# MattAgostini/ECE1782-Smith-Waterman-CUDA

Measured on AMD Instinct MI355X. Metric: GCUPS (DP cell updates/s) query-vs-SwissProt, 1/2/4/8 MI355X; bit-exact scores, higher is better.
Workload: dtype fp16

## Files before the change

ece1782-smith-waterman-cuda_amd/csrc/sw_capi.cpp:

```cpp
#include <algorithm>
#include <cmath>
#include <atomic>
#include <cstdio>
#include <cstdlib>
#include <cstring>
#include <memory>
#include <new>
#include <numeric>
#include <string>
#include <unordered_map>
#include <vector>

#include "sw_dbfile.h"
#include "sw_host.h"
#include "sw_pack.h"
#include "sw_parallel.h"
#include "sw_plan.h"
#include "sw_synth_host.h"

using swk::DevPtr;
using swk::Event;
using swk::HostPtr;
using swk::parallel_for;
using swk::Stream;
// ... 598 lines not shown
    const uint8_t* codes = nullptr;
    const sw_scoring* sc = nullptr;
    const sw_pssm* pssm = nullptr;
    int go = 0, ge = 0;
    int32_t qlen = 0;
};
QuerySrc seq_src(const uint8_t* q, int32_t qlen, const sw_scoring* sc) {
    QuerySrc s;
    s.codes = q;
    s.qlen = qlen;
    s.sc = sc;
    return s;
}
QuerySrc pssm_src(const sw_pssm* p, int32_t go, int32_t ge) {
    QuerySrc s;
    s.pssm = p;
    s.qlen = p ? p->qlen : 0;
    s.go = go;
    s.ge = ge;
    return s;
}
int check_pssm(const sw_handle* h, const sw_pssm* p, int go, int ge) {
    if (!h || !p) return fail(SW_E_INVALID, "null argument");
    if (p->h->device != h->device) return fail(SW_E_INVALID, "the PSSM was created on another handle's device");
    return check_gaps(go, ge);
}

struct Profiles {
    int8_t* dev = nullptr;
    int32_t stride = 0;
    size_t off8 = 0;
    size_t off16 = 0;
    size_t intra_off = 0;
    size_t total = 0;
    int slot = 0;
};

int build_profiles(sw_handle* h, const QuerySrc& src, const int8_t* mat, int go, bool affine,
                   int32_t qpad_inter, bool want16, int ri, int32_t qpad_intra, int32_t* const (&reset)[10],
                   Profiles* P) {
    const uint8_t* q = src.codes;
    const int32_t qlen = src.qlen;
    for (int32_t i = 0; i < qlen && !src.pssm; ++i)
        if (q[i] >= SW_ALPHABET) return fail(SW_E_INVALID, "query residue code out of range (use sw_encode)");
    const int bias = affine ? 0 : go;
    P->stride = static_cast<int32_t>(round_up(std::max<int32_t>(qpad_inter, 16), 16));
    const size_t n = static_cast<size_t>(swk::kProfileRows) * P->stride;
    size_t at = 0;
    auto take = [&](size_t bytes) {
        const size_t o = at;
        at = round_up(static_cast<int64_t>(at + bytes), 256);
        return o;
    };
    P->off8 = take(n);
    P->off16 = want16 ? take(2 * n) : 0;
    const int rip = swk::intra_rip(ri);
    const size_t intra_bytes = ri ? static_cast<size_t>(qpad_intra / (swk::kLanes * ri)) * swk::intra_chunk_bytes(ri) : 0;
    P->intra_off = take(intra_bytes);
    P->total = at;
    P->slot = h->prof_next;
    sw_handle::ProfSlot& S = h->prof[h->prof_next];
    h->prof_next = (h->prof_next + 1) % sw_handle::kProfSlots;
    if (S.pending) HIPCHECK(hipEventSynchronize(S.last_end));
    S.pending = false;
    if (P->total > S.dcap) {
        if (S.d.get()) {
            HIPCHECK(hipStreamSynchronize(h->stream.get()));
            if (S.tail_pending) HIPCHECK(hipEventSynchronize(S.tail_read.get()));
            S.tail_pending = false;
            S.d.reset();
        }
        S.dcap = std::max<size_t>(P->total, 1 << 16);
        HIPCHECK(swk::dev_alloc(S.d, S.dcap));
    }
    P->dev = S.d.get();
    if (S.tail_pending) {
        HIPCHECK(hipStreamWaitEvent(h->stream.get(), S.tail_read.get(), 0));
        S.tail_pending = false;
    }
    if (src.pssm) {
        swk::PssmProfileArgs a{};
        a.p8 = S.d.get() + P->off8;
        a.p16 = want16 ? reinterpret_cast<int16_t*>(S.d.get() + P->off16) : nullptr;
        a.pin = ri ? S.d.get() + P->intra_off : nullptr;
        a.stride = P->stride;
        a.qlen = qlen;
        a.bias = bias;
        a.ri = ri;
        a.rip = rip;
        a.qpad_intra = ri ? qpad_intra : 0;
        a.rows = std::max(P->stride, a.qpad_intra);
        for (int k = 0; k < 10; ++k) a.reset[k] = reset[k];
        a.pssm = src.pssm->d.get();
        a.ld = src.pssm->ld;
        HIPCHECK(swk::launch_build_profile_pssm(a, h->stream.get()));
        S.last_end = h->ev[3].get();
        S.pending = true;
        h->open_slot = P->slot;
        return SW_OK;
    }
    swk::ProfileArgs a{};
    a.p8 = S.d.get() + P->off8;
    a.p16 = want16 ? reinterpret_cast<int16_t*>(S.d.get() + P->off16) : nullptr;
    a.pin = ri ? S.d.get() + P->intra_off : nullptr;
    a.stride = P->stride;
    a.qlen = qlen;
    a.bias = bias;
    a.ri = ri;
    a.rip = rip;
    a.qpad_intra = ri ? qpad_intra : 0;
    for (int k = 0; k < 10; ++k) a.reset[k] = reset[k];
    std::memcpy(a.mat, mat, 625);
    const int32_t rows = std::max(P->stride, a.qpad_intra);
    for (int32_t r0 = 0; r0 < rows; r0 += swk::kProfQueryChunk) {
        a.row0 = r0;
        a.row1 = std::min(rows, r0 + swk::kProfQueryChunk);
        const int32_t nq = std::max(0, std::min(a.row1, qlen) - r0);
        if (nq) std::memcpy(a.q, q + r0, static_cast<size_t>(nq));
        HIPCHECK(swk::launch_build_profile(a, h->stream.get()));
        for (auto& p : a.reset) p = nullptr;
    }
    S.last_end = h->ev[3].get();
    S.pending = true;
    h->open_slot = P->slot;
    return SW_OK;
}

const sw_db::LptTable* lpt_table(sw_db* db, const swplan::ScanPlan& p) {
    const sw_opts& O = db->h->opts;
    const bool tri = p.ntri != 0;
    for (const auto& t : db->lay.lpt_tables)
        if (t.qpad == p.qpad_inter && t.rows == p.lpt_rows && t.qpad_intra == p.qpad_intra2 && t.ri == p.ri2 &&
            t.npair == p.npair && t.group == p.nquad && t.tail == p.ntail && t.pipe_opt == O.lpt_pipe &&
            t.affine == p.affine && t.tri == tri && t.tail_opt == O.lpt_pipe_tail)
            return &t;
    const swplan::LptPlan pl = swplan::lpt_plan(plan_view(db), p.qpad_inter, p.lpt_rows, p.qpad_intra2, p.ri2, p.npair,
                                                p.nquad, p.ntail, p.affine, tri);
    sw_db::LptTable t{p.qpad_inter, p.lpt_rows, p.qpad_intra2, p.ri2, p.npair, p.nquad, p.ntail,
                      static_cast<int32_t>(pl.order.size()), p.affine, tri, pl.npipe, O.lpt_pipe, pl.pipe_tail,
                      O.lpt_pipe_tail, DevPtr<int32_t>{}, pl.cost};
    const size_t bytes = pl.order.size() * sizeof(int32_t);
    hipError_t e = swk::dev_alloc(t.d_order, bytes);
    if (e == hipSuccess) e = hipMemcpy(t.d_order.get(), pl.order.data(), bytes, hipMemcpyHostToDevice);
// ... 177 lines not shown
    c.par = h->parity;
    h->parity ^= 1;
    if (h->tail_pending[c.par]) {
        HIPCHECK(hipStreamWaitEvent(h->stream.get(), h->tail_done[c.par].get(), 0));
        h->tail_pending[c.par] = false;
    }
    if (p.drain && (rc = join_tails(h))) return rc;
    if (db->lay.d_rescue.get()) {
        c.listA = db->lay.d_rescue.get() + c.par * rstride;
        c.listB = c.listA + db->shape.nblocks + 1;
        c.maxA = c.listA + 2 * (db->shape.nblocks + 1);
        c.headA = c.maxA + 2;
        if (p.lpt && h->opts.lpt_persist != 0) c.lpt_next = c.maxA + 1;
    }
    if (db->lay.d_lrescue.get()) {
        c.list1 = db->lay.d_lrescue.get() + c.par * lstride;
        c.list2 = c.list1 + db->shape.nlong + 1;
        c.head1 = c.list2 + db->shape.nlong + 1;
    }
    c.deferred = !p.drain && defer && (!(p.multi_inter || p.multi_intra) || ensure_rbnd(db, p.affine, p.intra_x2));
    return SW_OK;
}

int scan_profiles(Scan& c, const QuerySrc& src, const int8_t* mat) {
    const swplan::ScanPlan& p = c.plan;
    const bool d = p.drain;
    int32_t* const cA = (p.rescue && c.db->shape.nblocks) ? c.listA : nullptr;
    int32_t* const c1 = p.intra_x2 ? c.list1 : nullptr;
    int32_t* const reset[10] = {cA, (cA && p.f16) ? c.listB : nullptr, (cA && p.f16) ? c.maxA : nullptr, c1,
                                c1 ? c.list2 : nullptr, d ? c.headA : nullptr, d ? c.headA + 1 : nullptr,
                                d ? c.head1 : nullptr, d ? c.head1 + 1 : nullptr, c.lpt_next};
    const int rc = build_profiles(c.h, src, mat, c.sc.go, p.affine,
                                  std::max({p.qpad_inter, p.qpad_rescue, p.qpad_coop, p.qpad_list, p.qpad_intra2}),
                                  p.shape.x2s || p.intra_x2, p.ri, p.qpad_intra, reset, &c.P);
    c.h->evpool[c.h->nscans - 1].merged = p.lpt;
    return rc;
}

int inter_args(Scan& c) {
    sw_db* db = c.db;
    const swplan::ScanPlan& p = c.plan;
    const int go = c.sc.go, ge = c.sc.ge;
    swk::InterArgs& a = c.a;
    a.residues = db->lay.d_res.get();
    a.blk_off = db->lay.d_blk_off.get();
    a.blk_groups = db->lay.d_blk_groups.get();
    a.blk_cols = db->lay.d_blk_cols.get();
    a.lane_ids = db->lay.d_lane_ids.get();
    a.nblocks = static_cast<int32_t>(db->shape.nblocks);
    a.prof = c.P.dev + (p.shape.x2s ? c.P.off16 : c.P.off8);
    a.prof_stride = c.P.stride;
    a.qpad = p.qpad_inter;
    a.gap_open = go;
    a.gap_extend = ge;
    a.bnd_h = db->lay.d_bnd_h.get();
    a.bnd_f = db->lay.d_bnd_f.get();
    a.scores = c.scores;
    if (c.h->opts.trace_file[0]) {
        if (!db->lay.h_trace.get()) {
            db->lay.trace_entries = static_cast<size_t>(2 * db->shape.nblocks + db->shape.nlong + 8);
            HIPCHECK(swk::host_alloc(db->lay.h_trace, 32 * db->lay.trace_entries, hipHostMallocMapped));
            std::memset(db->lay.h_trace.get(), 0, 32 * db->lay.trace_entries);
        }
        HIPCHECK(hipHostGetDevicePointer(reinterpret_cast<void**>(&a.trace), db->lay.h_trace.get(), 0));
    }
    if (p.rescue) {
        a.rescue_count = c.listA;
        a.rescue_list = c.listA + 1;
        if (p.f16) a.rescue_max = c.maxA;
        const swplan::CellRange cr = swplan::cell_range(-128, c.sc.max_s, go, ge);
        a.sat_limit = cr.sat_limit;
        std::copy(std::begin(cr.step), std::end(cr.step), a.f16_step);
        a.f16_gog = cr.gog;
        a.f16_zero = cr.step[0];
        std::copy(std::begin(cr.diff), std::end(cr.diff), a.f16_diff);
    }
    a.re_last = p.re_last;
    if (p.lpt) {
        a.blk_first = p.npair;
        a.blk_quad = p.nquad;
        a.blk_tri = p.ntri ? 1 : 0;
        a.blk_tail = static_cast<int32_t>(db->shape.nblocks) - p.ntail;
    } else if (p.npair) {
        a.blk_base = p.nr;
        a.blk_first = std::max(p.npair, p.nr);
    } else {
        a.blk_first = p.ncoop;
    }
    return SW_OK;
}

void intra_args(Scan& c) {
    const sw_db* db = c.db;
    swk::IntraArgs& ia = c.ia;
    ia.residues = db->lay.d_lres.get();
    ia.subj_off = db->lay.d_loff.get();
    ia.subj_len = db->lay.d_llen.get();
    ia.subj_id = db->lay.d_lid.get();
    ia.nsubj = static_cast<int32_t>(db->shape.nlong);
    ia.prof = c.P.dev + c.P.intra_off;
    ia.qpad = c.plan.qpad_intra;
    ia.gap_open = c.sc.go;
    ia.gap_extend = c.sc.ge;
    ia.bnd_h = db->lay.d_lbnd_h.get();
    ia.bnd_f = db->lay.d_lbnd_f.get();
    ia.scores = c.scores;
}

void intra_x2_args(Scan& c) {
    const swplan::ScanPlan& p = c.plan;
// ... 1144 lines not shown
```

ece1782-smith-waterman-cuda_amd/csrc/sw_inter_x2.hip:

```cpp
#include <algorithm>

#include "sw_int32.h"
#include "sw_intra_x2.h"
#include "sw_kernels.h"

namespace swk {

typedef short s2 __attribute__((ext_vector_type(2)));
typedef unsigned short u2 __attribute__((ext_vector_type(2)));

__device__ __forceinline__ s2 as_s2(uint32_t x) { return __builtin_bit_cast(s2, x); }
__device__ __forceinline__ uint32_t as_u32(s2 x) { return __builtin_bit_cast(uint32_t, x); }
__device__ __forceinline__ s2 max2(s2 a, s2 b) { return __builtin_elementwise_max(a, b); }
__device__ __forceinline__ s2 usub2(s2 a, u2 g) {
    return __builtin_bit_cast(s2, __builtin_elementwise_sub_sat(__builtin_bit_cast(u2, a), g));
}

__host__ __device__ constexpr int x2_row_dwords(int R) { return (R / 4) % 2 == 1 ? R : R + 4; }

constexpr int kImgCodes = kPadCode + 1;

template <int R>
struct __attribute__((aligned(16))) X2Lds {
    static constexpr int kImg = kImgCodes * x2_row_dwords(R);
    uint32_t lo[kImg];
    uint32_t hi[kImg];
};
static_assert(sizeof(X2Lds<32>) % 16 == 0 && sizeof(X2Lds<48>) % 16 == 0, "image alignment");

template <int N>
__device__ __forceinline__ uint32_t word(const int4 (&v)[N], int w) {
    const int4 q = v[w >> 2];
    switch (w & 3) {
        case 0: return static_cast<uint32_t>(q.x);
        case 1: return static_cast<uint32_t>(q.y);
        case 2: return static_cast<uint32_t>(q.z);
        default: return static_cast<uint32_t>(q.w);
    }
}

template <int SG>
__device__ __forceinline__ void load_codes(uint32_t (&w)[SG / 4], const uint8_t* p, bool valid) {
    if (valid) {
        if constexpr (SG == 16) {
            const int4 v = *reinterpret_cast<const int4*>(p);
            w[0] = v.x; w[1] = v.y; w[2] = v.z; w[3] = v.w;
        } else if constexpr (SG == 8) {
            const int2 v = *reinterpret_cast<const int2*>(p);
            w[0] = v.x; w[1] = v.y;
        } else {
            w[0] = *reinterpret_cast<const uint32_t*>(p);
        }
    } else {
#pragma unroll
        for (int q = 0; q < SG / 4; ++q) w[q] = 0x19191919u;
    }
}

__device__ __forceinline__ uint32_t code_of(const uint32_t* w, int jj) { return (w[jj >> 2] >> (8 * (jj & 3))) & 0xffu; }

template <uint32_t RB>
// ... 26 lines not shown
__device__ __forceinline__ void load_bnd(uint32_t (&v)[SG], const uint32_t* bnd, uint64_t i) {
    if constexpr (AFFINE) {
        load_pairs<SG>(v, reinterpret_cast<const int32_t*>(bnd) + i);
    } else {
        const uint16_t* p = reinterpret_cast<const uint16_t*>(bnd) + i;
        uint32_t w[SG / 2];
        if constexpr (SG == 8) {
            const int4 t = *reinterpret_cast<const int4*>(p);
            w[0] = t.x; w[1] = t.y; w[2] = t.z; w[3] = t.w;
        } else {
            static_assert(SG == 4, "sub-group width");
            const int2 t = *reinterpret_cast<const int2*>(p);
            w[0] = t.x; w[1] = t.y;
        }
#pragma unroll
        for (int q = 0; q < SG; ++q) v[q] = w[q / 2];
    }
}
template <int SG, bool AFFINE>
__device__ __forceinline__ void store_bnd(uint32_t* bnd, uint64_t i, const uint32_t (&hb)[SG]) {
    if constexpr (AFFINE) {
        store_pairs<SG>(reinterpret_cast<int32_t*>(bnd) + i, hb);
    } else {
        uint16_t* p = reinterpret_cast<uint16_t*>(bnd) + i;
        uint32_t w[SG / 2];
#pragma unroll
        for (int q = 0; q < SG / 2; ++q) w[q] = lo_lo(hb[2 * q], hb[2 * q + 1]);
        if constexpr (SG == 8) *reinterpret_cast<int4*>(p) = make_int4(w[0], w[1], w[2], w[3]);
        else *reinterpret_cast<int2*>(p) = make_int2(w[0], w[1]);
    }
}


template <int R, bool F16>
__device__ __forceinline__ void stage_x2s(X2Lds<R>& L, const int16_t* __restrict__ prof, int stride, int s0,
                                          int lane, int bias, int bias0, int img, int hi0 = R) {
    constexpr int RD = x2_row_dwords(R);
    constexpr int PER = kImgCodes * (R / 8);
    constexpr uint32_t one = 1u;
    const int n = img < 0 ? 2 * PER : PER;
    for (int t = lane; t < n; t += kLanes) {
        const int im = img < 0 ? t / PER : img;
        const int u = img < 0 ? t % PER : t;
        const int c = u / (R / 8);
        const int k = u % (R / 8);
        const int16_t* src = prof + static_cast<size_t>(c) * stride + s0 + im * hi0 + 8 * k;
        int4 v;
        if (im && (hi0 & 7)) {
            const int2 v0 = *reinterpret_cast<const int2*>(src), v1 = *reinterpret_cast<const int2*>(src + 4);
            v = make_int4(v0.x, v0.y, v1.x, v1.y);
        } else {
            v = *reinterpret_cast<const int4*>(src);
        }
        const uint32_t w[4] = {static_cast<uint32_t>(v.x), static_cast<uint32_t>(v.y), static_cast<uint32_t>(v.z),
                               static_cast<uint32_t>(v.w)};
        uint32_t o[8];
#pragma unroll
        for (int e = 0; e < 4; ++e) {
            const int s0v = static_cast<int16_t>(w[e] & 0xffffu), s1v = static_cast<int16_t>(w[e] >> 16);
            const int b0 = (F16 && k % 2 == 0 && e == 0) ? bias0 : 0;
            const uint32_t a0 = static_cast<uint32_t>(s0v) & 0xffffu, a1 = static_cast<uint32_t>(s1v) & 0xffffu;
            if constexpr (F16) {
                const uint32_t w0 = static_cast<uint32_t>(s0v + bias + b0), w1 = static_cast<uint32_t>(s1v + bias);
                o[2 * e] = im ? w0 << 16 : w0;
                o[2 * e + 1] = im ? w1 << 16 : w1;
            } else {
                o[2 * e] = im ? (a0 << 16) | one : a0 | (one << 16);
                o[2 * e + 1] = im ? (a1 << 16) | one : a1 | (one << 16);
            }
        }
        int4* d = reinterpret_cast<int4*>((im ? L.hi : L.lo) + c * RD + 8 * k);
        d[0] = make_int4(o[0], o[1], o[2], o[3]);
        d[1] = make_int4(o[4], o[5], o[6], o[7]);
    }
}


typedef int v4i __attribute__((ext_vector_type(4)));
typedef __attribute__((address_space(3))) const v4i lds_int4;

__device__ __forceinline__ uint32_t lds_addr(const void* p) {
    return static_cast<uint32_t>(reinterpret_cast<uintptr_t>(p));
}

template <int N>
__device__ __forceinline__ void read_x2a(int4 (&pl)[N], int4 (&ph)[N], uint32_t& aa, uint32_t& ab, int k,
                                         uint32_t dep) {
    asm volatile("" : "+v"(aa), "+v"(ab) : "v"(dep));
    lds_int4* a = reinterpret_cast<lds_int4*>(static_cast<uintptr_t>(aa)) + N * k;
    lds_int4* b = reinterpret_cast<lds_int4*>(static_cast<uintptr_t>(ab)) + N * k;
#pragma unroll
    for (int q = 0; q < N; ++q) {
        pl[q] = __builtin_bit_cast(int4, a[q]);
        ph[q] = __builtin_bit_cast(int4, b[q]);
    }
}

typedef _Float16 h2 __attribute__((ext_vector_type(2)));

template <bool F16>
struct PkCell;

template <>
struct PkCell<false> {
    using V = s2;
    static __device__ __forceinline__ V from(uint32_t x) { return as_s2(x); }
// ... 154 lines not shown
};
__device__ __forceinline__ void pair_wait(const int* prog, int wave, int need) {
    while (__hip_atomic_load(prog + wave, __ATOMIC_ACQUIRE, __HIP_MEMORY_SCOPE_WORKGROUP) < need)
        __builtin_amdgcn_s_sleep(1);
}

template <int R, int SG, bool AFFINE, bool F16, bool PAIR, int CR = 16, bool CHAIN = false, int RL = R>
__device__ __forceinline__ void x2s_pass(const InterArgs& a, X2Lds<R>& L, uint32_t ncols, uint64_t base, int lane,
                                         int s0, Best<F16>& best, const int4* ring_in, int4* ring_out,
                                         int* tick, const PairSync* ps = nullptr, int chain_passes = 1) {
    static_assert(!(CHAIN && PAIR), "chained passes: single-wave blocks only");
    constexpr int CQ = CR / 4;
    constexpr int NCH = R / CR;
    constexpr int STEPS = SG * NCH;
    using P = PkCell<F16>;
    using V = typename P::V;
    const int16_t* prof16 = reinterpret_cast<const int16_t*>(a.prof);
    const u2 go2 = {static_cast<unsigned short>(a.gap_open), static_cast<unsigned short>(a.gap_open)};
    const u2 ge2 = {static_cast<unsigned short>(a.gap_extend), static_cast<unsigned short>(a.gap_extend)};
    uint32_t* bnd = reinterpret_cast<uint32_t*>(a.bnd_h);
    static_assert(!F16 || (R % kRowGroup == 0 && SG <= 8), "fp16 row groups");
    h2 gog_h = {}, reb_h = {}, grp_h = {};
    if constexpr (F16) {
        gog_h = __builtin_bit_cast(h2, a.f16_gog);
        static_assert(SG == 4 || SG == 8, "rebase constants");
        reb_h = __builtin_bit_cast(h2, a.f16_diff[SG == 4 ? 0 : 1]);
        grp_h = __builtin_bit_cast(h2, a.f16_diff[2]);
    }
    const bool first = (s0 == 0);
    const bool last = (s0 + 2 * R >= a.qpad);
    const uint32_t npass = CHAIN ? static_cast<uint32_t>(chain_passes) : 1u;
    const bool chain_last = CHAIN && static_cast<int>(npass) * 2 * R >= a.qpad;
    const uint32_t total = npass * ncols;
    const int sbias = F16 ? (AFFINE ? 2 : 1) * a.gap_extend : 0;
    const int gbias0 = F16 ? -kRowGroup * a.gap_extend : 0;
    const uint32_t dtop0 = F16 ? a.f16_step[SG - 2 + kRowGroup] : 0u;
    constexpr bool kSh = RL < R;
    if constexpr (kSh) asm volatile("" : "+v"(lane));
    static_assert(!kSh || (RL == R - 4 && !CHAIN), "rows per strip: R, or R - 4 outside a chain");
    static_assert((R - 4 - 1) % kRowGroup == 11, "the short strip's bottom row: 4 ge under the last row's bias");
    h2 dsh_h = {};
    if constexpr (F16) dsh_h = __builtin_bit_cast(h2, a.f16_diff[0]);
    stage_x2s<R, F16>(L, prof16, a.prof_stride, s0, lane, sbias, gbias0, -1, RL);
    __builtin_amdgcn_fence(__ATOMIC_RELEASE, "workgroup");
    __builtin_amdgcn_wave_barrier();
    __builtin_amdgcn_fence(__ATOMIC_ACQUIRE, "workgroup");

    V H[R];
    V E[AFFINE ? R : 1];
#pragma unroll
    for (int r = 0; r < R; ++r) H[r] = P::from(F16 && r < RL ? a.f16_step[r % kRowGroup + SG - 1] : 0u);
#pragma unroll
    for (int r = 0; r < (AFFINE ? R : 1); ++r) E[r] = P::from(F16 ? a.f16_zero : 0u);
    uint32_t dtop = dtop0;
    uint32_t dl_h[SG], dl_f[SG];
    uint32_t bin[SG], bin_n[SG];
    uint32_t bz[SG];
    uint32_t rc[SG / 4], rp[SG / 4], rn[SG / 4];
#pragma unroll
    for (int q = 0; q < SG; ++q) {
        bz[q] = !F16 ? 0u
                     : AFFINE ? lo_lo(a.f16_step[kRowGroup - 1 + q], a.f16_step[kRowGroup + q])
                              : lo_lo(a.f16_step[kRowGroup - 1 + q], a.f16_step[kRowGroup - 1 + q]);
        dl_h[q] = F16 ? a.f16_step[kRowGroup - 1 + q] : 0u;
        dl_f[q] = F16 ? a.f16_step[kRowGroup + q] : 0u;
        bin[q] = bz[q];
        bin_n[q] = 0;
    }
#pragma unroll
    for (int q = 0; q < SG / 4; ++q) rp[q] = 0x19191919u;
    load_codes<SG>(rc, a.residues + base, true);
    constexpr bool kPairFlags = pair_flags<AFFINE>();
    auto wait_in = [&](uint32_t x) {
        if constexpr (PAIR && kPairFlags)
            pair_wait(ps->prog, ps->pred, ps->pred_base + min(static_cast<int>(x) + 2, ps->S));
    };
    if (!first) {
        wait_in(0);
        if (PAIR && ring_in) ring_load<SG>(bin, ring_in, 0, lane);
        else load_bnd<SG, AFFINE>(bin, bnd, base);
    }
    int4 PL[2][CQ], PH[2][CQ];
    constexpr uint32_t RB = x2_row_dwords(R) * 4;
    const uint32_t blo = lds_addr(L.lo), bhi = lds_addr(L.hi);
    uint32_t aa = code_row<RB>(rc, 0, blo), ab = bhi + kPadCode * RB;
    read_x2a<CQ>(PL[0], PH[0], aa, ab, 0, 0);

    uint32_t lo_p = 0, lo_c = 0;
    bool t2 = false;
    for (uint32_t col0 = 0; col0 <= total; col0 += SG) {
        const bool has_next = col0 + SG <= total;
        const bool next_lo = col0 + SG < total;
        const uint32_t ncol = col0 + SG;
        const bool wrap = CHAIN && lo_c + SG == ncols;
        const uint32_t nreal = CHAIN ? (wrap ? 0u : lo_c + SG) : ncol;
        const bool next_first = CHAIN ? (lo_p == 0 && !wrap) : first;
        const uint64_t noff = (nreal >> 4) * kGroupBytes + (nreal & 15);
        const bool t1 = CHAIN && lo_c == 0 && lo_p > 0 && lo_p < npass;
        const bool next_t1 = CHAIN && wrap && next_lo;
        const bool next_t2 = t1;
        if (t1) {
            stage_x2s<R, F16>(L, prof16, a.prof_stride, static_cast<int>(lo_p) * 2 * R, lane, sbias, gbias0, 0);
#pragma unroll
            for (int r = 0; r < R; ++r) {
                H[r] = P::from(__builtin_amdgcn_perm(P::bits(H[r]), F16 ? a.f16_step[r % kRowGroup + SG - 1] : 0u,
                                                     0x07060100u));
                if constexpr (AFFINE) E[r] = P::from(__builtin_amdgcn_perm(P::bits(E[r]), F16 ? a.f16_zero : 0u, 0x07060100u));
            }
            dtop = __builtin_amdgcn_perm(dtop, dtop0, 0x07060100u);
        }
        if (t2) {
            stage_x2s<R, F16>(L, prof16, a.prof_stride, static_cast<int>(lo_p) * 2 * R, lane, sbias, gbias0, 1);
#pragma unroll
            for (int r = 0; r < R; ++r) {
                H[r] = P::from(__builtin_amdgcn_perm(F16 ? a.f16_step[r % kRowGroup + SG - 1] : 0u, P::bits(H[r]),
                                                     0x07060100u));
                if constexpr (AFFINE) E[r] = P::from(__builtin_amdgcn_perm(F16 ? a.f16_zero : 0u, P::bits(E[r]), 0x07060100u));
            }
            dtop = __builtin_amdgcn_perm(dtop0, dtop, 0x07060100u);
        }
        if (t1 || t2) {
            __builtin_amdgcn_fence(__ATOMIC_RELEASE, "workgroup");
            __builtin_amdgcn_wave_barrier();
            __builtin_amdgcn_fence(__ATOMIC_ACQUIRE, "workgroup");
            aa = code_row<RB>(rc, 0, blo);
            ab = code_row<RB>(rp, 0, bhi);
            read_x2a<CQ>(PL[0], PH[0], aa, ab, 0, 0);
        }
        if (next_t1) {
            __builtin_amdgcn_fence(__ATOMIC_RELEASE, "workgroup");
            __builtin_amdgcn_fence(__ATOMIC_ACQUIRE, "workgroup");
        }
        if (has_next) {
            load_codes<SG>(rn, a.residues + base + noff, next_lo);
            if (!next_first && next_lo) {
                wait_in(ncol / SG);
                if (PAIR && ring_in) ring_load<SG>(bin_n, ring_in, (ncol / SG) % kRingSlots, lane);
                else load_bnd<SG, AFFINE>(bin_n, bnd, base + noff);
            }
        }
        if constexpr (F16) {
#pragma unroll
            for (int r = 0; r < R; ++r) {
                if (r < RL) H[r] = isub(H[r], reb_h);
                if constexpr (AFFINE)
                    if (r < RL) E[r] = isub(E[r], reb_h);
            }
            dtop -= P::bits(reb_h);
        }
        auto cell = [&](const int r, const int jj, V& up, V& diag, V& f, const V slo, const V shi) {
            if constexpr (F16 && !AFFINE) {
                const int rg = r % kRowGroup;
                if (rg == 0 && r > 0) up = isub(up, grp_h);
                const h2 t = max3h(H[r], up, iadd(iadd(slo, shi), diag));
                const h2 h = __builtin_elementwise_maximum(t, __builtin_bit_cast(h2, a.f16_step[rg + jj]));
                h2& acc = best.acc[rg + jj];
                if (jj & 1) {
                    if (rg + 1 < kRowGroup) acc = max3h(acc, h, H[r + 1]);
                    else acc = __builtin_elementwise_maximum(acc, h);
                } else if (rg == 0) {
                    acc = __builtin_elementwise_maximum(acc, h);
                }
                diag = H[r];
                H[r] = h;
                up = h;
            } else if constexpr (!AFFINE) {
                const s2 h = usub2(max2(max2(H[r], up), slo * shi + diag), go2);
                diag = H[r];
                H[r] = h;
                up = h;
                best.v = max2(best.v, h);
            } else if constexpr (!F16) {
                const s2 h = max2(max2(E[r], f), slo * shi + diag);
                const s2 n = usub2(h, go2);
                E[r] = max2(usub2(E[r], ge2), n);
                f = max2(usub2(f, ge2), n);
                diag = H[r];
                H[r] = h;
                up = h;
                best.v = max2(best.v, h);
            }
        };
        auto cell_d = [&](const int r, const int jj, V& up, V& diag, V& f, const V d) {
          if constexpr (F16 && AFFINE) {
            const int rg = r % kRowGroup;
            if (rg == 0 && r > 0) f = isub(f, grp_h);
            const h2 h = max3h(E[r], f, d);
            const h2 m = isub(h, gog_h);
            E[r] = __builtin_elementwise_maximum(E[r], m);
            f = max3h(f, m, __builtin_bit_cast(h2, a.f16_step[rg + jj + 1]));
            h2& acc = best.acc[rg + jj];
            if (jj & 1) {
                if (rg + 1 < kRowGroup) acc = max3h(acc, h, H[r + 1]);
                else acc = __builtin_elementwise_maximum(acc, h);
            } else if (rg == 0) {
                acc = __builtin_elementwise_maximum(acc, h);
            }
            diag = H[r];
            H[r] = h;
            up = h;
          }
        };
        auto col_done = [&](const V up, const V f, const int jj) {
            if constexpr (kSh && F16) {
                dl_h[jj] = P::bits(iadd(up, dsh_h));
                if constexpr (AFFINE) dl_f[jj] = P::bits(iadd(f, dsh_h));
            } else {
                dl_h[jj] = P::bits(up);
                if constexpr (AFFINE) dl_f[jj] = P::bits(f);
            }
        };
        auto col_start = [&](V& up, V& diag, V& f, const int jj) {
            const uint32_t u = (AFFINE || jj % 2 == 0) ? lo_lo(bin[jj], dl_h[jj]) : hi_lo(bin[jj], dl_h[jj]);
            up = P::from(u);
            if constexpr (F16 && !AFFINE) up = isub(up, grp_h);
            diag = P::from(dtop);
            dtop = u;
            if constexpr (AFFINE) f = P::from(hi_lo(bin[jj], dl_f[jj]));
            if constexpr (F16) f = isub(f, grp_h);
        };
        V up = P::from(0u), diag = P::from(0u), f = P::from(0u);
#pragma unroll
        for (int t = 0; t < STEPS; ++t) {
            const int jj = t / NCH;
            const int k = t % NCH;
            const uint32_t dep = P::bits(k == 0 ? H[R - 1] : H[CR * k - 1]);
            if (t + 1 < STEPS) {
                const int jn = (t + 1) / NCH, kn = (t + 1) % NCH;
                if (kn == 0) {
                    aa = code_row<RB>(rc, jn, blo);
// ... 465 lines not shown
```

ece1782-smith-waterman-cuda_amd/csrc/sw_kernels.h:

```cpp
#pragma once

#include <hip/hip_runtime.h>
#include <stdint.h>

#include <string>

#include "sw_amd.h"

namespace swk {

int set_error(int code, const std::string& msg);

constexpr int kLanes = 64;
constexpr int kGroupCols = 16;
constexpr int kGroupBytes = kLanes * kGroupCols;
constexpr int kProfileRows = 32;
constexpr int kPadCode = 25;
constexpr uint8_t kStored[26] = {11, 1, 5, 2, 22, 6, 14, 12, 23, 9, 10, 0, 24, 7, 4, 15, 3, 21, 8, 13, 16, 17, 18, 19, 20, 25};
constexpr uint8_t kCodeOf[26] = {11, 1, 3, 16, 14, 2, 5, 13, 18, 9, 10, 0, 7, 19, 6, 15, 20, 21, 22, 23, 24, 17, 4, 8, 12, 25};
constexpr int kWavesPerWG = 4;
constexpr int kIntraSteps = 40;

template <int SG>
struct Residues {
    uint32_t w[SG / 4];
    __device__ __forceinline__ void load(const uint8_t* p) {
        if constexpr (SG == 16) {
            const int4 v = *reinterpret_cast<const int4*>(p);
            w[0] = v.x; w[1] = v.y; w[2] = v.z; w[3] = v.w;
        } else if constexpr (SG == 8) {
            const int2 v = *reinterpret_cast<const int2*>(p);
            w[0] = v.x; w[1] = v.y;
        } else {
            w[0] = *reinterpret_cast<const uint32_t*>(p);
        }
    }
    __device__ __forceinline__ uint32_t code(int jj) const { return (w[jj >> 2] >> (8 * (jj & 3))) & 0xffu; }
};

struct InterArgs {
    const uint8_t* residues;
    const uint64_t* blk_off;
    const uint32_t* blk_groups;
    const uint32_t* blk_cols;
    const int32_t* lane_ids;
    int32_t nblocks;
    const int8_t* prof;
    int32_t prof_stride;
    int32_t qpad;
    int32_t gap_open;
    int32_t gap_extend;
    int32_t* bnd_h;
    int32_t* bnd_f;
    int32_t* scores;
    int32_t* rescue_list;
    int32_t* rescue_count;
    const int32_t* blk_list;
    const int32_t* blk_count;
    int32_t blk_first;
    int32_t sat_limit;
    uint32_t f16_step[32];
    uint32_t f16_gog;
    uint32_t f16_zero;
    uint32_t f16_diff[3];
    int32_t blk_base;
    int32_t blk_quad;
    int32_t blk_tri;
    int32_t blk_tail;
    int32_t* rescue_max;
    uint64_t* trace;
    int32_t re_last;
};

struct IntraArgs {
    const uint8_t* residues;
    const uint64_t* subj_off;
    const int32_t* subj_len;
    const int32_t* subj_id;
    int32_t nsubj;
    const int8_t* prof;
    int32_t qpad;
    int32_t gap_open;
    int32_t gap_extend;
    int32_t* bnd_h;
    int32_t* bnd_f;
    int32_t* scores;
    int32_t prof_stride = 0;
    int32_t bias = 0;
    int32_t sat_limit = 0;
    uint32_t f16_step[kIntraSteps] = {};
    uint32_t f16_zero = 0;
    uint32_t f16_gog = 0;
    int32_t* rescue_list = nullptr;
    int32_t* rescue_count = nullptr;
    const int32_t* subj_list = nullptr;
    const int32_t* list_count = nullptr;
    int32_t pipe_pairs = 0;
    int32_t pipe_tail = 0x7fffffff;
};

#if defined(__HIPCC__)
__device__ __forceinline__ int tid_x() {
    int t = static_cast<int>(threadIdx.x);
    asm volatile("" : "+v"(t));
// ... 100 lines not shown
    int64_t ops_stride;
};
hipError_t launch_align(const AlignArgs& a, hipStream_t s);

struct SynthFill {
    uint8_t* res;
    const uint64_t* blk_off;
    const uint32_t* blk_groups;
    const int32_t* lane_local;
    const int32_t* lane_len;
    int64_t nblocks;
    uint8_t* lres;
    const uint64_t* loff;
    const int32_t* llen;
    const int32_t* lid;
    int32_t nlong;
    uint64_t seed;
    int64_t id_base;
    const uint8_t* lut;
};
hipError_t launch_synth_fill(const SynthFill& f, hipStream_t s);

constexpr int kAlphabet = 25;
constexpr int kProfQueryChunk = 2048;
struct ProfileArgs {
    int8_t* p8;
    int16_t* p16;
    int8_t* pin;
    int32_t stride;
    int32_t qlen;
    int32_t row0, row1;
    int32_t bias;
    int32_t ri, rip, qpad_intra;
    int32_t* reset[10];
    int8_t mat[kAlphabet * kAlphabet + 15];
    uint8_t q[kProfQueryChunk];
};
hipError_t launch_build_profile(const ProfileArgs& a, hipStream_t s);
struct PssmProfileArgs {
    int8_t* p8;
    int16_t* p16;
    int8_t* pin;
    int32_t stride;
    int32_t qlen;
    int32_t rows;
    int32_t bias;
    int32_t ri, rip, qpad_intra;
    int32_t* reset[10];
    const int8_t* pssm;
    int32_t ld;
};
hipError_t launch_build_profile_pssm(const PssmProfileArgs& a, hipStream_t s);

struct TopkSrc {
    const int32_t* scores;
    const int64_t* keys;
    const int32_t* rid;
    const int32_t* gid;
    int64_t id_base;
};
size_t topk_workspace_bytes(int64_t n, int k);
hipError_t launch_topk(const TopkSrc& src, int64_t n, int k, int64_t* out, int64_t* work, hipStream_t s);

}
```

ece1782-smith-waterman-cuda_amd/csrc/sw_plan.cpp:

```cpp
#include "sw_plan.h"

#include <algorithm>
#include <cmath>
#include <cstdio>
#include <utility>
#include <vector>

namespace swplan {

namespace {
int32_t round_up(int64_t v, int64_t m) { return static_cast<int32_t>((v + m - 1) / m * m); }
}


constexpr int64_t kSmallDbSubjects = 64 * 1000;

constexpr double kFillSubjects = 570000.0;

int32_t default_long_threshold(const PlanDb& db) {
    if (db.n == 0) return 1536;
    const double mean = static_cast<double>(db.residues) / static_cast<double>(db.n);
    if (db.n < kSmallDbSubjects && mean >= 256) return 64;
    const double fill = db.n < kSmallDbSubjects ? 1.0 : std::min(1.0, static_cast<double>(db.n) / kFillSubjects);
    const double t = 5.7 * mean * std::pow(fill, 0.4);
// ... 318 lines not shown
    p.lpt_rows = (p.lpt && !affine && O.lpt_rows != 64 && round_up(qlen, 96) > 96) ? 96 : 64;
    p.qpad_inter = round_up(qlen, p.lpt_rows == 96 ? 96 : R);
    p.re_last = p.shape.x2s ? short_rows(qlen, p.lpt_rows == 96 ? 96 : R) : 0;
    if (p.lpt) {
        const int passes = p.qpad_inter / p.lpt_rows;
        p.ntri = affine ? lpt_tri_blocks(db, p.npair, passes) : 0;
        p.nquad = p.ntri ? p.ntri : lpt_quad_blocks(db, p.npair);
        p.ntail = lpt_tail_blocks(db, p.npair, passes);
    }

    p.ri = db.nlong ? intra_rows_for(qlen, db.long_max) : 0;
    p.qpad_intra = p.ri ? round_up(qlen, static_cast<int64_t>(swk::kLanes) * p.ri) : 0;
    p.ri2 = p.lpt ? ri2_lpt : ri2_model;
    p.qpad_intra2 = p.ri2 ? round_up(qlen, static_cast<int64_t>(swk::kLanes) * p.ri2) : 0;
    p.multi_inter = p.qpad_inter > R || p.qpad_rescue > rescue_rows(affine) || p.qpad_coop > swk::kCoopRows ||
                    p.qpad_list > list_rows;
    p.multi_intra = (p.ri && p.qpad_intra > swk::kLanes * p.ri) || (p.ri2 && p.qpad_intra2 > swk::kLanes * p.ri2);

    if (db.nblocks) {
        p.kernel = inter_kernel_name(p.shape, affine);
        if (p.npair) p.kernel.replace(0, sizeof("sw_inter_x2s") - 1, "sw_inter_x2p");
        if (p.lpt_rows == 96) p.kernel.replace(p.kernel.find("<32,"), 4, "<48,");
        if (p.nr) p.kernel += "+int16[0," + std::to_string(p.nr) + ")";
        if (p.ntail) p.kernel += "+tail" + std::to_string(p.ntail);
        if (p.ntri) p.kernel += "+tri" + std::to_string(p.ntri);
        if (p.lpt) p.kernel += "+lpt";
    }
    p.intra_kernel = !db.nlong   ? "none"
                     : p.intra_x2 ? "sw_intra_x2<" + std::to_string(p.ri2) + (p.intra_i16_first ? ",int16>" : ">")
                                  : "sw_intra<" + std::to_string(p.ri) + (affine ? ",affine>" : ",linear>");
    return p;
}

void ScanPlan::set_drain(bool got_rows) {
    if (!lpt || !got_rows || drain) return;
    drain = true;
    ri = ri2;
    qpad_intra = qpad_intra2;
    multi_intra = qpad_intra > swk::kLanes * ri;
    kernel += "+drain";
}

}
```

ece1782-smith-waterman-cuda_amd/csrc/sw_plan.h:

```cpp
#pragma once

#include <cstdint>
#include <string>
#include <vector>

#include "sw_amd.h"
#include "sw_kernels.h"

namespace swplan {

struct PlanDb {
    int64_t n = 0;
    int64_t residues = 0;
    int64_t nblocks = 0;
    int64_t nlong = 0;
    int32_t long_threshold = 0;
    int32_t long_max = 0;
    const uint32_t* blk_groups = nullptr;
    const int32_t* llen = nullptr;
    const sw_opts* opts = nullptr;
    int cus = 0;
};

int32_t default_long_threshold(const PlanDb& db);
// ... 34 lines not shown
    bool intra_i16_first = false;
    int ri = 0;
    int ri2 = 0;
    int32_t qpad_inter = 0, qpad_intra = 0, qpad_intra2 = 0, qpad_rescue = 0, qpad_list = 0, qpad_coop = 0;
    int32_t npair = 0;
    int32_t ncoop = 0;
    int32_t nr = 0;
    bool lpt = false;
    bool drain = false;
    int lpt_rows = 64;
    int32_t re_last = 0;
    int32_t ntri = 0, nquad = 0, ntail = 0;
    bool multi_inter = false, multi_intra = false;
    std::string kernel, intra_kernel;

    void set_drain(bool got_rows);
};

constexpr int kCellMin = 0x0400, kCellMax = 0x7BFF;
struct CellRange {
    int z = 0;
    uint32_t step[32] = {};
    uint32_t gog = 0;
    uint32_t diff[3] = {};
    int sat_limit = 0;
    int lowest = 0;
    int guard = 0;
    int top = 0;
};
CellRange cell_range(int min_s, int max_s, int go, int ge);

ScanPlan scan_plan(const PlanDb& db, int32_t qlen, const PlanScoring& s, bool intra_i16_first, int32_t i16_span);

struct LptPlan {
    std::vector<int32_t> order;
    std::vector<float> cost;
    int32_t npipe = 0;
    int32_t pipe_tail = 0;
};
LptPlan lpt_plan(const PlanDb& db, int32_t qpad, int rows, int32_t qpad_intra, int ri, int32_t npair, int32_t nquad,
                 int32_t ntail, bool affine, bool tri);

}
```

ece1782-smith-waterman-cuda_amd/csrc/sw_profile.hip:

```cpp
#include "sw_kernels.h"

namespace swk {

template <class A>
__device__ __forceinline__ void profile_reset(const A& a) {
    if (blockIdx.x == 0 && threadIdx.x < 10) {
        int32_t* p = a.reset[threadIdx.x];
        if (p) *p = threadIdx.x == 2 ? -1 : 0;
    }
}

template <class A>
__device__ __forceinline__ void profile_store(const A& a, int c, int i, int v) {
    if (i < a.stride) {
        const size_t k = static_cast<size_t>(c) * a.stride + i;
        a.p8[k] = static_cast<int8_t>(v);
        if (a.p16) a.p16[k] = static_cast<int16_t>(v);
    }
    if (a.pin && i < a.qpad_intra) {
        const int ch = i / (kLanes * a.ri), w = i % (kLanes * a.ri);
        const int t = w / a.ri, r = w % a.ri;
        int8_t* d = a.pin + ((static_cast<size_t>(ch) * kProfileRows + c) * kLanes + t) * a.rip;
        d[r] = static_cast<int8_t>(v);
        if (r == a.ri - 1)
            for (int p = a.ri; p < a.rip; ++p) d[p] = 0;
    }
}

__global__ __launch_bounds__(256) void sw_build_profile(ProfileArgs a) {
    profile_reset(a);
    const int n = a.row1 - a.row0;
    const int tid = blockIdx.x * blockDim.x + threadIdx.x;
    if (tid >= kProfileRows * n) return;
    const int c = tid / n;
    const int i = a.row0 + tid % n;
    const int v =
        (c >= kAlphabet || i >= a.qlen) ? a.bias : a.mat[kAlphabet * a.q[i - a.row0] + kCodeOf[c]] + a.bias;
    profile_store(a, c, i, v);
}

__global__ __launch_bounds__(256) void sw_build_profile_pssm(PssmProfileArgs a) {
    profile_reset(a);
    const int64_t tid = static_cast<int64_t>(blockIdx.x) * blockDim.x + threadIdx.x;
    if (tid >= static_cast<int64_t>(kProfileRows) * a.rows) return;
    const int c = static_cast<int>(tid / a.rows);
    const int i = static_cast<int>(tid % a.rows);
    const int8_t* __restrict__ t = a.pssm;
    const int v = (c >= kAlphabet || i >= a.qlen) ? a.bias : t[static_cast<size_t>(kCodeOf[c]) * a.ld + i] + a.bias;
    profile_store(a, c, i, v);
}

// ... 17 lines not shown
```

Before: 11610.

## Prebuild biased fp16 pass images in profile kernel and copy them into LDS

For the F16 x2s inter kernel, the profile-build kernel now writes per-pass LDS images (biased, packed 16-bit words) into device memory once per query. The inter kernel then copies these images straight into LDS with vector loads, several in flight, instead of rebuilding them from the int16 profile with bias arithmetic on every stage. This moves per-block staging work into a single precompute, at the cost of extra device memory and a larger profile kernel. Edge-row max accumulation is also reorganised into a helper lambda.

```diff
diff --git a/ece1782-smith-waterman-cuda_amd/csrc/sw_capi.cpp b/ece1782-smith-waterman-cuda_amd/csrc/sw_capi.cpp
--- a/ece1782-smith-waterman-cuda_amd/csrc/sw_capi.cpp
+++ b/ece1782-smith-waterman-cuda_amd/csrc/sw_capi.cpp
@@ -654,13 +654,15 @@
     size_t off8 = 0;
     size_t off16 = 0;
     size_t intra_off = 0;
+    size_t img_off = 0;
+    bool img = false;
     size_t total = 0;
     int slot = 0;
 };
 
 int build_profiles(sw_handle* h, const QuerySrc& src, const int8_t* mat, int go, bool affine,
-                   int32_t qpad_inter, bool want16, int ri, int32_t qpad_intra, int32_t* const (&reset)[10],
-                   Profiles* P) {
+                   int32_t qpad_inter, bool want16, int ri, int32_t qpad_intra, const swk::PassImages& images,
+                   int32_t* const (&reset)[10], Profiles* P) {
     const uint8_t* q = src.codes;
     const int32_t qlen = src.qlen;
     for (int32_t i = 0; i < qlen && !src.pssm; ++i)
@@ -679,6 +681,8 @@
     const int rip = swk::intra_rip(ri);
     const size_t intra_bytes = ri ? static_cast<size_t>(qpad_intra / (swk::kLanes * ri)) * swk::intra_chunk_bytes(ri) : 0;
     P->intra_off = take(intra_bytes);
+    P->img = images.R > 0;
+    P->img_off = P->img ? take(swk::pass_img_bytes(images)) : 0;
     P->total = at;
     P->slot = h->prof_next;
     sw_handle::ProfSlot& S = h->prof[h->prof_next];
@@ -711,6 +715,10 @@
         a.ri = ri;
         a.rip = rip;
         a.qpad_intra = ri ? qpad_intra : 0;
+        if (P->img) {
+            a.img = images;
+            a.img.words = reinterpret_cast<uint32_t*>(S.d.get() + P->img_off);
+        }
         a.rows = std::max(P->stride, a.qpad_intra);
         for (int k = 0; k < 10; ++k) a.reset[k] = reset[k];
         a.pssm = src.pssm->d.get();
@@ -731,6 +739,10 @@
     a.ri = ri;
     a.rip = rip;
     a.qpad_intra = ri ? qpad_intra : 0;
+    if (P->img) {
+        a.img = images;
+        a.img.words = reinterpret_cast<uint32_t*>(S.d.get() + P->img_off);
+    }
     for (int k = 0; k < 10; ++k) a.reset[k] = reset[k];
     std::memcpy(a.mat, mat, 625);
     const int32_t rows = std::max(P->stride, a.qpad_intra);
@@ -974,7 +986,8 @@
                                 d ? c.head1 : nullptr, d ? c.head1 + 1 : nullptr, c.lpt_next};
     const int rc = build_profiles(c.h, src, mat, c.sc.go, p.affine,
                                   std::max({p.qpad_inter, p.qpad_rescue, p.qpad_coop, p.qpad_list, p.qpad_intra2}),
-                                  p.shape.x2s || p.intra_x2, p.ri, p.qpad_intra, reset, &c.P);
+                                  p.shape.x2s || p.intra_x2, p.ri, p.qpad_intra,
+                                  c.db->shape.nblocks ? swplan::pass_images(p, c.sc.ge) : swk::PassImages{}, reset, &c.P);
     c.h->evpool[c.h->nscans - 1].merged = p.lpt;
     return rc;
 }
@@ -1018,6 +1031,7 @@
         std::copy(std::begin(cr.diff), std::end(cr.diff), a.f16_diff);
     }
     a.re_last = p.re_last;
+    a.img = c.P.img ? reinterpret_cast<const uint32_t*>(c.P.dev + c.P.img_off) : nullptr;
     if (p.lpt) {
         a.blk_first = p.npair;
         a.blk_quad = p.nquad;
diff --git a/ece1782-smith-waterman-cuda_amd/csrc/sw_inter_x2.hip b/ece1782-smith-waterman-cuda_amd/csrc/sw_inter_x2.hip
--- a/ece1782-smith-waterman-cuda_amd/csrc/sw_inter_x2.hip
+++ b/ece1782-smith-waterman-cuda_amd/csrc/sw_inter_x2.hip
@@ -3,6 +3,7 @@
 #include "sw_int32.h"
 #include "sw_intra_x2.h"
 #include "sw_kernels.h"
+#include "sw_pass_images.h"
 
 namespace swk {
 
@@ -16,9 +17,8 @@
     return __builtin_bit_cast(s2, __builtin_elementwise_sub_sat(__builtin_bit_cast(u2, a), g));
 }
 
-__host__ __device__ constexpr int x2_row_dwords(int R) { return (R / 4) % 2 == 1 ? R : R + 4; }
-
-constexpr int kImgCodes = kPadCode + 1;
+constexpr int kImgCodes = kPassImgCodes;
+static_assert(kImgCodes == kPadCode + 1, "image codes");
 
 template <int R>
 struct __attribute__((aligned(16))) X2Lds {
@@ -27,6 +27,9 @@
     uint32_t hi[kImg];
 };
 static_assert(sizeof(X2Lds<32>) % 16 == 0 && sizeof(X2Lds<48>) % 16 == 0, "image alignment");
+static_assert(sizeof(X2Lds<32>) == pass_img_slot_dwords(32) * 4 && sizeof(X2Lds<48>) == pass_img_slot_dwords(48) * 4 &&
+                  offsetof(X2Lds<32>, hi) == pass_img_dwords(32) * 4 && offsetof(X2Lds<48>, hi) == pass_img_dwords(48) * 4,
+              "prebuilt image layout");
 
 template <int N>
 __device__ __forceinline__ uint32_t word(const int4 (&v)[N], int w) {
@@ -119,9 +122,9 @@
 }
 
 
-template <int R, bool F16>
+template <int R>
 __device__ __forceinline__ void stage_x2s(X2Lds<R>& L, const int16_t* __restrict__ prof, int stride, int s0,
-                                          int lane, int bias, int bias0, int img, int hi0 = R) {
+                                          int lane, int img, int hi0 = R) {
     constexpr int RD = x2_row_dwords(R);
     constexpr int PER = kImgCodes * (R / 8);
     constexpr uint32_t one = 1u;
@@ -144,21 +147,34 @@
         uint32_t o[8];
 #pragma unroll
         for (int e = 0; e < 4; ++e) {
-            const int s0v = static_cast<int16_t>(w[e] & 0xffffu), s1v = static_cast<int16_t>(w[e] >> 16);
-            const int b0 = (F16 && k % 2 == 0 && e == 0) ? bias0 : 0;
-            const uint32_t a0 = static_cast<uint32_t>(s0v) & 0xffffu, a1 = static_cast<uint32_t>(s1v) & 0xffffu;
-            if constexpr (F16) {
-                const uint32_t w0 = static_cast<uint32_t>(s0v + bias + b0), w1 = static_cast<uint32_t>(s1v + bias);
-                o[2 * e] = im ? w0 << 16 : w0;
-                o[2 * e + 1] = im ? w1 << 16 : w1;
-            } else {
-                o[2 * e] = im ? (a0 << 16) | one : a0 | (one << 16);
-                o[2 * e + 1] = im ? (a1 << 16) | one : a1 | (one << 16);
-            }
+            const uint32_t a0 = w[e] & 0xffffu, a1 = w[e] >> 16;
+            o[2 * e] = im ? (a0 << 16) | one : a0 | (one << 16);
+            o[2 * e + 1] = im ? (a1 << 16) | one : a1 | (one << 16);
         }
         int4* d = reinterpret_cast<int4*>((im ? L.hi : L.lo) + c * RD + 8 * k);
         d[0] = make_int4(o[0], o[1], o[2], o[3]);
         d[1] = make_int4(o[4], o[5], o[6], o[7]);
+    }
+}
+
+template <int R, int N>
+__device__ __forceinline__ void copy_x2s(X2Lds<R>& L, const uint32_t* __restrict__ imgs, int slot, int lane, int img) {
+    constexpr int PER = pass_img_dwords(R) / 4;
+    const int4* __restrict__ src =
+        reinterpret_cast<const int4*>(imgs + static_cast<size_t>(slot) * pass_img_slot_dwords(R)) + (img > 0 ? PER : 0);
+    int4* dst = reinterpret_cast<int4*>(img > 0 ? L.hi : L.lo);
+    const int n = img < 0 ? 2 * PER : PER;
+    static_assert(N == 2 || N == 4, "loads in flight");
+    for (int t = lane; t < n; t += N * kLanes) {
+        const int t1 = min(t + kLanes, n - 1), t2 = min(t + 2 * kLanes, n - 1), t3 = min(t + 3 * kLanes, n - 1);
+        const int4 v0 = src[t], v1 = src[t1];
+        if constexpr (N == 4) {
+            const int4 v2 = src[t2], v3 = src[t3];
+            dst[t2] = v2;
+            dst[t3] = v3;
+        }
+        dst[t] = v0;
+        dst[t1] = v1;
     }
 }
 
@@ -379,8 +395,7 @@
     const uint32_t npass = CHAIN ? static_cast<uint32_t>(chain_passes) : 1u;
     const bool chain_last = CHAIN && static_cast<int>(npass) * 2 * R >= a.qpad;
     const uint32_t total = npass * ncols;
-    const int sbias = F16 ? (AFFINE ? 2 : 1) * a.gap_extend : 0;
-    const int gbias0 = F16 ? -kRowGroup * a.gap_extend : 0;
+    static_assert(kRowGroup == kPassImgGroup, "row groups");
     const uint32_t dtop0 = F16 ? a.f16_step[SG - 2 + kRowGroup] : 0u;
     constexpr bool kSh = RL < R;
     if constexpr (kSh) asm volatile("" : "+v"(lane));
@@ -388,7 +403,8 @@
     static_assert((R - 4 - 1) % kRowGroup == 11, "the short strip's bottom row: 4 ge under the last row's bias");
     h2 dsh_h = {};
     if constexpr (F16) dsh_h = __builtin_bit_cast(h2, a.f16_diff[0]);
-    stage_x2s<R, F16>(L, prof16, a.prof_stride, s0, lane, sbias, gbias0, -1, RL);
+    if constexpr (F16) copy_x2s<R, 4>(L, a.img, kSh ? a.qpad / (2 * R) : s0 / (2 * R), lane, -1);
+    else stage_x2s<R>(L, prof16, a.prof_stride, s0, lane, -1, RL);
     __builtin_amdgcn_fence(__ATOMIC_RELEASE, "workgroup");
     __builtin_amdgcn_wave_barrier();
     __builtin_amdgcn_fence(__ATOMIC_ACQUIRE, "workgroup");
@@ -447,7 +463,8 @@
         const bool next_t1 = CHAIN && wrap && next_lo;
         const bool next_t2 = t1;
         if (t1) {
-            stage_x2s<R, F16>(L, prof16, a.prof_stride, static_cast<int>(lo_p) * 2 * R, lane, sbias, gbias0, 0);
+            if constexpr (F16) copy_x2s<R, 2>(L, a.img, static_cast<int>(lo_p), lane, 0);
+            else stage_x2s<R>(L, prof16, a.prof_stride, static_cast<int>(lo_p) * 2 * R, lane, 0);
 #pragma unroll
             for (int r = 0; r < R; ++r) {
                 H[r] = P::from(__builtin_amdgcn_perm(P::bits(H[r]), F16 ? a.f16_step[r % kRowGroup + SG - 1] : 0u,
@@ -457,7 +474,8 @@
             dtop = __builtin_amdgcn_perm(dtop, dtop0, 0x07060100u);
         }
         if (t2) {
-            stage_x2s<R, F16>(L, prof16, a.prof_stride, static_cast<int>(lo_p) * 2 * R, lane, sbias, gbias0, 1);
+            if constexpr (F16) copy_x2s<R, 2>(L, a.img, static_cast<int>(lo_p), lane, 1);
+            else stage_x2s<R>(L, prof16, a.prof_stride, static_cast<int>(lo_p) * 2 * R, lane, 1);
 #pragma unroll
             for (int r = 0; r < R; ++r) {
                 H[r] = P::from(__builtin_amdgcn_perm(F16 ? a.f16_step[r % kRowGroup + SG - 1] : 0u, P::bits(H[r]),
@@ -495,6 +513,12 @@
             }
             dtop -= P::bits(reb_h);
         }
+        auto edge_max = [&](h2& acc, const h2 h, const int r) {
+            if constexpr (F16) {
+                if ((r / kRowGroup) % 2 == 1) acc = max3h(acc, H[r >= kRowGroup ? r - kRowGroup : 0], h);
+                else if (r + kRowGroup >= RL) acc = __builtin_elementwise_maximum(acc, h);
+            }
+        };
         auto cell = [&](const int r, const int jj, V& up, V& diag, V& f, const V slo, const V shi) {
             if constexpr (F16 && !AFFINE) {
                 const int rg = r % kRowGroup;
@@ -502,12 +526,8 @@
                 const h2 t = max3h(H[r], up, iadd(iadd(slo, shi), diag));
                 const h2 h = __builtin_elementwise_maximum(t, __builtin_bit_cast(h2, a.f16_step[rg + jj]));
                 h2& acc = best.acc[rg + jj];
-                if (jj & 1) {
-                    if (rg + 1 < kRowGroup) acc = max3h(acc, h, H[r + 1]);
-                    else acc = __builtin_elementwise_maximum(acc, h);
-                } else if (rg == 0) {
-                    acc = __builtin_elementwise_maximum(acc, h);
-                }
+                if ((jj & 1) && rg + 1 < kRowGroup) acc = max3h(acc, h, H[r + 1]);
+                else if ((jj & 1) || rg == 0) edge_max(acc, h, r);
                 diag = H[r];
                 H[r] = h;
                 up = h;
@@ -537,12 +557,8 @@
             E[r] = __builtin_elementwise_maximum(E[r], m);
             f = max3h(f, m, __builtin_bit_cast(h2, a.f16_step[rg + jj + 1]));
             h2& acc = best.acc[rg + jj];
-            if (jj & 1) {
-                if (rg + 1 < kRowGroup) acc = max3h(acc, h, H[r + 1]);
-                else acc = __builtin_elementwise_maximum(acc, h);
-            } else if (rg == 0) {
-                acc = __builtin_elementwise_maximum(acc, h);
-            }
+            if ((jj & 1) && rg + 1 < kRowGroup) acc = max3h(acc, h, H[r + 1]);
+            else if ((jj & 1) || rg == 0) edge_max(acc, h, r);
             diag = H[r];
             H[r] = h;
             up = h;
diff --git a/ece1782-smith-waterman-cuda_amd/csrc/sw_kernels.h b/ece1782-smith-waterman-cuda_amd/csrc/sw_kernels.h
--- a/ece1782-smith-waterman-cuda_amd/csrc/sw_kernels.h
+++ b/ece1782-smith-waterman-cuda_amd/csrc/sw_kernels.h
@@ -6,6 +6,7 @@
 #include <string>
 
 #include "sw_amd.h"
+#include "sw_pass_images.h"
 
 namespace swk {
 
@@ -70,6 +71,7 @@
     int32_t* rescue_max;
     uint64_t* trace;
     int32_t re_last;
+    const uint32_t* img;
 };
 
 struct IntraArgs {
@@ -236,6 +238,7 @@
     int32_t row0, row1;
     int32_t bias;
     int32_t ri, rip, qpad_intra;
+    PassImages img;
     int32_t* reset[10];
     int8_t mat[kAlphabet * kAlphabet + 15];
     uint8_t q[kProfQueryChunk];
@@ -250,6 +253,7 @@
     int32_t rows;
     int32_t bias;
     int32_t ri, rip, qpad_intra;
+    PassImages img;
     int32_t* reset[10];
     const int8_t* pssm;
     int32_t ld;
diff --git a/ece1782-smith-waterman-cuda_amd/csrc/sw_pass_images.h b/ece1782-smith-waterman-cuda_amd/csrc/sw_pass_images.h
--- /dev/null
+++ b/ece1782-smith-waterman-cuda_amd/csrc/sw_pass_images.h
@@ -0,0 +1,56 @@
+#pragma once
+
+#include <hip/hip_runtime.h>
+#include <stddef.h>
+#include <stdint.h>
+
+namespace swk {
+
+__host__ __device__ constexpr int x2_row_dwords(int R) { return (R / 4) % 2 == 1 ? R : R + 4; }
+
+constexpr int kPassImgCodes = 26;
+constexpr int kPassImgGroup = 16;
+
+struct PassImages {
+    uint32_t* words = nullptr;
+    int32_t R = 0;
+    int32_t passes = 0;
+    int32_t re_last = 0;
+    int32_t bias = 0;
+    int32_t bias0 = 0;
+};
+
+__host__ __device__ constexpr int pass_img_dwords(int R) { return kPassImgCodes * x2_row_dwords(R); }
+__host__ __device__ constexpr int pass_img_slot_dwords(int R) { return 2 * pass_img_dwords(R); }
+__host__ __device__ inline int pass_img_slots(const PassImages& g) { return g.passes + (g.re_last == g.R - 4 ? 1 : 0); }
+__host__ __device__ inline size_t pass_img_bytes(const PassImages& g) {
+    return static_cast<size_t>(pass_img_slots(g)) * pass_img_slot_dwords(g.R) * sizeof(uint32_t);
+}
+
+__host__ __device__ inline size_t pass_img_index(int R, int slot, int image, int code, int row) {
+    return (static_cast<size_t>(slot) * 2 + image) * pass_img_dwords(R) + code * x2_row_dwords(R) + row;
+}
+
+__host__ __device__ inline int pass_img_row(const PassImages& g, int slot, int image, int row) {
+    if (slot < g.passes) return slot * 2 * g.R + image * g.R + row;
+    return (g.passes - 1) * 2 * g.R + image * (g.R - 4) + row;
+}
+
+__host__ __device__ inline uint32_t pass_img_word(const PassImages& g, int image, int row, int v) {
+    const uint32_t w = static_cast<uint32_t>(v + g.bias + (row % kPassImgGroup == 0 ? g.bias0 : 0));
+    return image ? w << 16 : w;
+}
+
+template <class F>
+__host__ __device__ inline void pass_img_for_row(const PassImages& g, int i, F f) {
+    const int R = g.R;
+    if (i < 0 || i >= g.passes * 2 * R) return;
+    const int p = i / (2 * R), o = i % (2 * R);
+    f(p, o / R, o % R);
+    if (pass_img_slots(g) > g.passes && p == g.passes - 1) {
+        if (o < R) f(g.passes, 0, o);
+        if (o >= R - 4 && o - (R - 4) < R) f(g.passes, 1, o - (R - 4));
+    }
+}
+
+}
diff --git a/ece1782-smith-waterman-cuda_amd/csrc/sw_plan.cpp b/ece1782-smith-waterman-cuda_amd/csrc/sw_plan.cpp
--- a/ece1782-smith-waterman-cuda_amd/csrc/sw_plan.cpp
+++ b/ece1782-smith-waterman-cuda_amd/csrc/sw_plan.cpp
@@ -374,6 +374,17 @@
     return p;
 }
 
+swk::PassImages pass_images(const ScanPlan& p, int ge) {
+    swk::PassImages g;
+    if (!p.f16 || !p.shape.x2s || p.qpad_inter <= 0) return g;
+    g.R = p.lpt_rows == 96 ? 48 : 32;
+    g.passes = p.qpad_inter / (2 * g.R);
+    g.re_last = p.re_last;
+    g.bias = (p.affine ? 2 : 1) * ge;
+    g.bias0 = -swk::kPassImgGroup * ge;
+    return g;
+}
+
 void ScanPlan::set_drain(bool got_rows) {
     if (!lpt || !got_rows || drain) return;
     drain = true;
diff --git a/ece1782-smith-waterman-cuda_amd/csrc/sw_plan.h b/ece1782-smith-waterman-cuda_amd/csrc/sw_plan.h
--- a/ece1782-smith-waterman-cuda_amd/csrc/sw_plan.h
+++ b/ece1782-smith-waterman-cuda_amd/csrc/sw_plan.h
@@ -90,6 +90,8 @@
 
 ScanPlan scan_plan(const PlanDb& db, int32_t qlen, const PlanScoring& s, bool intra_i16_first, int32_t i16_span);
 
+swk::PassImages pass_images(const ScanPlan& p, int ge);
+
 struct LptPlan {
     std::vector<int32_t> order;
     std::vector<float> cost;
diff --git a/ece1782-smith-waterman-cuda_amd/csrc/sw_profile.hip b/ece1782-smith-waterman-cuda_amd/csrc/sw_profile.hip
--- a/ece1782-smith-waterman-cuda_amd/csrc/sw_profile.hip
+++ b/ece1782-smith-waterman-cuda_amd/csrc/sw_profile.hip
@@ -17,6 +17,10 @@
         a.p8[k] = static_cast<int8_t>(v);
         if (a.p16) a.p16[k] = static_cast<int16_t>(v);
     }
+    if (a.img.words && c < kPassImgCodes)
+        pass_img_for_row(a.img, i, [&](int slot, int image, int row) {
+            a.img.words[pass_img_index(a.img.R, slot, image, c, row)] = pass_img_word(a.img, image, row, v);
+        });
     if (a.pin && i < a.qpad_intra) {
         const int ch = i / (kLanes * a.ri), w = i % (kLanes * a.ri);
         const int t = w / a.ri, r = w % a.ri;
```

Result: no change. 11660, median of 6 (+0.4%).
